# noamzilo/sed-crnn

Measured on AMD Instinct MI355X. Metric: mel-frames/sec training throughput (seq=256, mel=40), higher is better.
Workload: dtype f32; 1 GPU; BASELINE config 2: mono (B=128,256,40,1) per GPU, 3xConv3x3(128)+BN+ReLU+pool(1,2)+dropout0.5, BiGRU 2x128, Linear(256,1), BCEWithLogits, Adam lr 1e-3; full fit step (fwd+loss+bwd+allreduce+Adam); global_batch=128, seq_len=256, n_mels=40, parallelism=single

## Files before the change

### include/sedcrnn.h

```cpp
#ifndef SEDCRNN_H
#define SEDCRNN_H

#include <stddef.h>
#include <stdint.h>

#ifdef __cplusplus
extern "C" {
#endif

#define SED_MAX_CONV 4
#define SED_MAX_GRU 4
#define SED_MAX_DENSE 4

int sed_version(void);
const char* sed_last_error_string(void);

int sed_conv3x3_pack_weights(const float* w_oihw, float* wp_fwd, float* wp_dgrad,
                             int Cout, int Cin, void* stream);

int sed_conv3x3_stat_rows(int B, int Cin, int F, int T, int Cout, int x_is_nchw);

int sed_conv3x3_plan(int B, int Cin, int F, int T, int Cout, int x_is_nchw, int which, int* out);

int sed_conv3x3_fwd(const float* x, int x_is_nchw, const float* wp, const float* bias,
// ... 130 lines not shown
                        void* workspace, int B, int Cin, int F, int T, int C, float drop_p,
                        const float* gamma, const float* beta, float* dgamma, void* stream);
int sed_conv1_bwd_wgrad_assemble(const float* partials, int rows, const double* moments, const float* wp, const float* bias,
                                 const float* mean, const float* rstd, const float* scale, const float* sum_g,
                                 const float* sum_gx, float* dw_oihw, float* dbias, int B, int Cin, int F, int T, int C,
                                 const float* gamma, const float* beta, float* dgamma, void* stream);

int sed_gemm_f32(const float* A, long a_si, long a_sk, const float* B, long b_sk, long b_sj,
                 float* C, long ldc, const float* bias, float beta, int M, int N, int K, void* stream);
size_t sed_gemm_f32_workspace_bytes(int M, int N, int K);
int sed_gemm_f32_ws(const float* A, long a_si, long a_sk, const float* B, long b_sk, long b_sj,
                    float* C, long ldc, const float* bias, int M, int N, int K, void* workspace, void* stream);

int sed_gemm_bf16_nt(const void* A, const void* B, const float* bias, float* C, long ldc, int M, int N, int K, void* stream);

int sed_gemm_f32_wgrad(const float* A, long a_si, long a_sk, const float* B, long b_sk, long b_sj,
                       float* C, long ldc, int M, int N, int K, void* workspace, void* stream);
int sed_gemm_f32_plan(int M, int N, int K, int policy, int* bm, int* bn, int* splits, int* k_len);

int sed_linear_fwd(const float* x, const float* W, const float* b, float* y,
                   int M, int K, int N, int relu, void* stream);
size_t sed_linear_bwd_workspace_bytes(int M, int K, int N);
int sed_linear_bwd(const float* x, const float* W, const float* y, float* dy, float* dx,
                   float* dW, float* db, void* workspace, int M, int K, int N, int relu, void* stream);

size_t sed_gru_seq_workspace_bytes(int H);
int sed_gru_seq_fwd(const float* gi, const float* const* whh, const float* const* bhh,
                    float* out, float* saved, void* workspace, int B, int T, int H, void* stream);
size_t sed_gru_seq_bwd_workspace_bytes(int B, int H);
int sed_gru_seq_bwd(const float* dout, const float* saved, const float* const* whh,
                    float* dgi, float* dgh, float* const* dbih, float* const* dbhh, void* workspace,
                    int B, int T, int H, void* stream);
int sed_gru_seq_variant(int B, int H, int* bt, int* hreg, int* hlds);

int sed_loss_fwd_bwd(const float* logits, const float* targets, int n, int kind, float alpha,
                     float gamma, int reduction_mean, float* loss, float* dlogits, float* probs,
                     void* stream);
int sed_sigmoid(const float* x, float* y, int n, void* stream);
int sed_scale(float* x, long n, float alpha, void* stream);

size_t sed_sqnorm_workspace_bytes(long n);
int sed_grad_norm_clip_coef(const float* g, long n, float max_norm, float* norm_out,
                            void* workspace, void* stream);
int sed_adam_step(float* p, const float* g, float* m, float* v, long n, float lr, float beta1,
                  float beta2, float eps, float weight_decay, int step, const float* grad_scale,
                  const uint64_t* step_state, void* stream);
int sed_step_advance(uint64_t* step_state, void* stream);

size_t sed_logmel_tables_bytes(const float* melfb_host, int n_fft, int n_mels);
int sed_logmel_build_tables(const float* window_host, const float* melfb_host, int n_fft, int n_mels,
                            void* tables_host, size_t tables_bytes);
int sed_logmel(const float* pcm, long n_samples, const void* tables, size_t tables_bytes,
               const float* mu, const float* inv_sigma, float* out,
               int n_fft, int hop, int n_mels, int pad_mode, void* stream);
size_t sed_logmel_batch_workspace_bytes(int R);
int sed_logmel_batch(const float* pcm, long pcm_len, const long* clips_host, int R, const void* tables, size_t tables_bytes,
                     const float* mu, const float* inv_sigma, float* out, long out_rows, int n_fft, int hop, int n_mels,
                     int pad_mode, void* workspace, size_t workspace_bytes, void* stream);
size_t sed_logmel_multi_workspace_bytes(int R, int channels);
int sed_logmel_multi(const float* pcm, long pcm_len, const long* clips_host, int R, int channels, const void* tables,
                     size_t tables_bytes, const float* mu, const float* inv_sigma, float* out, long out_rows, int n_fft, int hop,
                     int n_mels, int pad_mode, void* workspace, size_t workspace_bytes, void* stream);
size_t sed_logmel_gcc_workspace_bytes(int R, int channels);
int sed_logmel_gcc(const float* pcm, long pcm_len, const long* clips_host, int R, int channels, const void* tables,
                   size_t tables_bytes, const float* mu, const float* inv_sigma, float* out, long out_rows, int n_fft, int hop,
                   int n_mels, int n_lags, int pad_mode, void* workspace, size_t workspace_bytes, void* stream);
// ... 327 lines not shown
```

### sed_crnn_amd/_lib.py

```python
import ctypes as C
import os

HERE = os.path.dirname(os.path.abspath(__file__))
LIB_PATH = os.environ.get("SED_CRNN_LIB") or os.path.join(HERE, "libsedcrnn.so")

SED_MAX_CONV = 4
SED_MAX_GRU = 4
SED_MAX_DENSE = 4

_fp = C.c_void_p
_stream = C.c_void_p


class NetCfg(C.Structure):
    _fields_ = [
        ("B", C.c_int), ("Cin", C.c_int), ("F", C.c_int), ("T", C.c_int),
        ("n_conv", C.c_int),
        ("C", C.c_int * SED_MAX_CONV),
        ("pool_f", C.c_int * SED_MAX_CONV), ("pool_t", C.c_int * SED_MAX_CONV),
        ("drop_p", C.c_float * SED_MAX_CONV),
        ("n_gru", C.c_int), ("H", C.c_int * SED_MAX_GRU),
        ("n_dense", C.c_int), ("D", C.c_int * SED_MAX_DENSE),
        ("bn_eps", C.c_float), ("bn_momentum", C.c_float),
        ("conv_mode", C.c_int),
# ... 64 lines not shown
    "sed_conv1_bwd_wgrad_assemble": (_i, [_fp, _i, _fp, _fp, _fp, _fp, _fp, _fp, _fp, _fp, _fp, _fp, _i, _i, _i, _i, _i, _fp, _fp, _fp, _stream]),
    "sed_conv1_route": (_i, [_fp, _fp, _fp, _fp, _fp, _fp, _i, _i, _i, _i, _i, _i, _i, _stream]),
    "sed_conv1_bwd_reduce": (_i, [_fp, _fp, _fp, _fp, _fp, _fp, _fp, _fp, _fp, _i, _i, _i, _i, _i, _i, _i, _f, _u64, _fp, _stream]),
    "sed_conv1_bwd_apply_workspace_bytes": (_sz, [_i, _i, _i, _i]),
    "sed_conv1_bwd_apply_wgrad": (_i, [_fp, _fp, _fp, _fp, _fp, _fp, _fp, _fp, _fp, _fp, _fp, _fp, _fp, _i, _i, _i, _i, _i, _i, _i, _f, _u64, _fp, _fp, _fp, _fp, _stream]),
    "sed_bn_finalize_train": (_i, [_fp, _i, _i, _d, _fp, _fp, _fp, _fp, _f, _f, _fp, _fp, _fp, _fp, _stream]),
    "sed_bn_stat_sums": (_i, [_fp, _i, _i, _fp, _stream]),
    "sed_bn_finalize_from_sums": (_i, [_fp, _i, _d, _fp, _fp, _fp, _fp, _f, _f, _fp, _fp, _fp, _fp, _stream]),
    "sed_bn_finalize_eval": (_i, [_fp, _fp, _fp, _fp, _f, _i, _fp, _fp, _stream]),
    "sed_bn_relu_pool_drop_fwd": (_i, [_fp, _fp, _fp, _fp, _i, _i, _i, _i, _i, _i, _i, _f, _u64, _fp, _stream]),
    "sed_bn_relu_pool_route": (_i, [_fp, _fp, _fp, _fp, _i, _i, _i, _i, _i, _i, _stream]),
    "sed_bn_bwd_rows": (_i, [_i, _i, _i]),
    "sed_bn_relu_pool_drop_bwd_reduce": (_i, [_fp, _fp, _fp, _fp, _fp, _fp, _fp, _i, _i, _i, _i, _i, _i, _i, _f, _u64, _fp, _stream]),
    "sed_bn_bwd_finalize": (_i, [_fp, _i, _i, _fp, _fp, _fp, _fp, _stream]),
    "sed_bn_bwd_finalize_small_gamma": (_i, [_fp, _i, _i, _fp, _fp, _fp, _fp, _fp, _fp, _fp, _fp, _fp, _fp, _fp, _fp, _fp, _i, _i, _i, _i, _i, _f, _stream]),
    "sed_bn_bwd_reduce_pooled_supported": (_i, [_i, _i, _i, _i, _i]),
    "sed_bn_bwd_reduce_pooled": (_i, [_fp, _fp, _fp, _fp, _fp, _fp, _fp, _fp, _fp, _fp, _i, _i, _i, _i, _i, _i, _i, _f, _stream]),
    "sed_bn_relu_pool_drop_bwd_apply": (_i, [_fp, _fp, _fp, _fp, _fp, _fp, _fp, _fp, _fp, _fp, _i, _i, _i, _i, _i, _i, _i, _f, _u64, _fp, _stream]),
    "sed_reduce_rows": (_i, [_fp, _i, _i, _i, _fp, _stream]),
    "sed_gemm_f32": (_i, [_fp, _l, _l, _fp, _l, _l, _fp, _l, _fp, _f, _i, _i, _i, _stream]),
    "sed_gemm_f32_workspace_bytes": (_sz, [_i, _i, _i]),
    "sed_gemm_f32_ws": (_i, [_fp, _l, _l, _fp, _l, _l, _fp, _l, _fp, _i, _i, _i, _fp, _stream]),
    "sed_gemm_bf16_nt": (_i, [_fp, _fp, _fp, _fp, _l, _i, _i, _i, _stream]),
    "sed_gemm_f32_wgrad": (_i, [_fp, _l, _l, _fp, _l, _l, _fp, _l, _i, _i, _i, _fp, _stream]),
    "sed_gemm_f32_plan": (_i, [_i, _i, _i, _i, C.POINTER(_i), C.POINTER(_i), C.POINTER(_i), C.POINTER(_i)]),
    "sed_linear_fwd": (_i, [_fp, _fp, _fp, _fp, _i, _i, _i, _i, _stream]),
    "sed_linear_bwd_workspace_bytes": (_sz, [_i, _i, _i]),
    "sed_linear_bwd": (_i, [_fp, _fp, _fp, _fp, _fp, _fp, _fp, _fp, _i, _i, _i, _i, _stream]),
    "sed_gru_seq_workspace_bytes": (_sz, [_i]),
    "sed_gru_seq_fwd": (_i, [_fp, _pp, _pp, _fp, _fp, _fp, _i, _i, _i, _stream]),
    "sed_gru_seq_bwd_workspace_bytes": (_sz, [_i, _i]),
    "sed_gru_seq_bwd": (_i, [_fp, _fp, _pp, _fp, _fp, _pp, _pp, _fp, _i, _i, _i, _stream]),
    "sed_gru_seq_variant": (_i, [_i, _i, C.POINTER(_i), C.POINTER(_i), C.POINTER(_i)]),
    "sed_loss_fwd_bwd": (_i, [_fp, _fp, _i, _i, _f, _f, _i, _fp, _fp, _fp, _stream]),
    "sed_sigmoid": (_i, [_fp, _fp, _i, _stream]),
    "sed_scale": (_i, [_fp, _l, _f, _stream]),
    "sed_sqnorm_workspace_bytes": (_sz, [_l]),
    "sed_grad_norm_clip_coef": (_i, [_fp, _l, _f, _fp, _fp, _stream]),
    "sed_adam_step": (_i, [_fp, _fp, _fp, _fp, _l, _f, _f, _f, _f, _f, _i, _fp, _fp, _stream]),
    "sed_step_advance": (_i, [_fp, _stream]),
    "sed_logmel_tables_bytes": (_sz, [_fp, _i, _i]),
    "sed_logmel_build_tables": (_i, [_fp, _fp, _i, _i, _fp, _sz]),
    "sed_logmel": (_i, [_fp, _l, _fp, _sz, _fp, _fp, _fp, _i, _i, _i, _i, _stream]),
    "sed_logmel_batch_workspace_bytes": (_sz, [_i]),
    "sed_logmel_batch": (_i, [_fp, _l, _fp, _i, _fp, _sz, _fp, _fp, _fp, _l, _i, _i, _i, _i, _fp, _sz, _stream]),
    "sed_logmel_multi_workspace_bytes": (_sz, [_i, _i]),
    "sed_logmel_multi": (_i, [_fp, _l, _fp, _i, _i, _fp, _sz, _fp, _fp, _fp, _l, _i, _i, _i, _i, _fp, _sz, _stream]),
    "sed_logmel_gcc_workspace_bytes": (_sz, [_i, _i]),
    "sed_logmel_gcc": (_i, [_fp, _l, _fp, _i, _i, _fp, _sz, _fp, _fp, _fp, _l, _i, _i, _i, _i, _i, _fp, _sz, _stream]),
    "sed_event_tdoa_workspace_bytes": (_sz, [_i, _i, _l, _l, _i, _i]),
    "sed_event_tdoa": (_i, [_fp, _l, _fp, _i, _i, _fp, _sz, _fp, _fp, _fp, _fp, _l, _i, _i, _i, _i, _i, _fp, _fp, _fp, _fp, _fp, _sz,
                            _stream]),
    "sed_stream_ring_write_workspace_bytes": (_sz, [_i]),
    "sed_stream_ring_write": (_i, [_fp, _l, _i, _l, _fp, _l, _fp, _fp, _sz, _stream]),
    "sed_event_tdoa_ring_workspace_bytes": (_sz, [_i, _i, _l, _l, _i, _i]),
    "sed_event_tdoa_ring": (_i, [_fp, _l, _l, _fp, _i, _i, _fp, _sz, _fp, _fp, _fp, _fp, _l, _i, _i, _i, _i, _i, _i, _fp, _fp, _fp, _fp,
                                 _fp, _sz, _stream]),
    "sed_event_doa_workspace_bytes": (_sz, [_i, _i, _l, _l, _i, _i]),
    "sed_event_doa": (_i, [_fp, _l, _fp, _i, _i, _fp, _sz, _fp, _fp, _fp, _fp, _l, _i, _i, _i, _i, _i, _fp, _fp, _fp, _fp, _fp, _i, _i,
                           _fp, _fp, _fp, _fp, _fp, _sz, _stream]),
    "sed_event_doa_ring_workspace_bytes": (_sz, [_i, _i, _l, _l, _i, _i]),
    "sed_event_doa_ring": (_i, [_fp, _l, _l, _fp, _i, _i, _fp, _sz, _fp, _fp, _fp, _fp, _l, _i, _i, _i, _i, _i, _i, _fp, _fp, _fp, _fp,
                                _fp, _i, _i, _fp, _fp, _fp, _fp, _fp, _sz, _stream]),
    "sed_event_doa_track_workspace_bytes": (_sz, [_i, _i, _l, _l, _i, _i, _i, _i, _i]),
    "sed_event_doa_track": (_i, [_fp, _l, _fp, _i, _i, _fp, _sz, _fp, _fp, _fp, _fp, _l, _i, _i, _i, _i, _i, _fp, _fp, _fp, _fp, _fp, _i,
                                 _i, _fp, _fp, _fp, _fp, _i, _fp, _fp, _fp, _fp, _fp, _fp, _fp, _fp, _sz, _stream]),
# ... 140 lines not shown
```

### sed_crnn_amd/csrc/gru.hip

```cpp
#include "common.h"

static inline int gru_bt(int H, int B) {
    int bt = B >= 512 ? 4 : (B >= 256 ? 2 : 1);
    if (H >= 128 && bt > 2) bt = 2;
    return bt;
}

__global__ void gru_pack_whh_t_k(const float* __restrict__ w0, const float* __restrict__ w1,
                                 float* __restrict__ wt, int H) {
    int i = blockIdx.x * blockDim.x + threadIdx.x;
    int n = 3 * H * H;
    if (i >= 2 * n) return;
    int dir = i / n, e = i - dir * n;
    int g = e / H, k = e - g * H;
    const float* w = dir ? w1 : w0;
    wt[(size_t)dir * n + (size_t)k * 3 * H + g] = w[e];
}

constexpr int gru_nt(int hreg) { return hreg > 0 ? ((3 * hreg + 63) / 64) * 64 : 1024; }

__device__ __forceinline__ float gru_dot4(float w0, float w1, float w2, float w3, const f32x4& h) {
    return fmaf(w3, h[3], fmaf(w2, h[2], fmaf(w0, h[0], w1 * h[1])));
}

template <int HREG, int GRU_BT, int HTOT = HREG, int HLDS = 0>
__global__ __launch_bounds__(gru_nt(HTOT)) void gru_seq_fwd_k(
    const float* __restrict__ gi, const float* __restrict__ wt, const float* __restrict__ bhh0,
    const float* __restrict__ bhh1, float* __restrict__ out, float* __restrict__ saved, int B, int T, int H) {
    extern __shared__ __attribute__((aligned(16))) float smem[];
    float* h_s = smem;
    float* gh_s = smem + GRU_BT * H;
    float* w_l = smem + GRU_BT * 4 * H;
    const int g = threadIdx.x;
    const int dir = blockIdx.y, b0 = blockIdx.x * GRU_BT;
    const int H3 = 3 * H;
    const float* wtd = wt + (size_t)dir * H3 * H;
    const float* bhh = dir ? bhh1 : bhh0;
    const bool row = g < H3;
    const bool gate = g < H;
    constexpr bool HYB = HTOT != HREG && HREG > 0;

    float wreg[HREG > 0 ? HREG : 1];
    if (HREG > 0 && row) {
#pragma unroll
        for (int k = 0; k < HREG; ++k) wreg[k] = wtd[(size_t)k * H3 + g];
    }
    if (HYB && row) {
        for (int j = 0; j < HLDS; ++j) w_l[j * H3 + g] = wtd[(size_t)(HREG + j) * H3 + g];
    }
    const float bias = row ? bhh[g] : 0.f;
    for (int i = g; i < GRU_BT * H; i += blockDim.x) h_s[i] = 0.f;
    __syncthreads();

    float gr[GRU_BT], gz[GRU_BT], gn[GRU_BT], nr[GRU_BT], nz[GRU_BT], nn[GRU_BT], mr[GRU_BT], mz[GRU_BT], mn[GRU_BT];
    auto fetch_gi = [&](int s, float* a, float* bq, float* c) {
        const int tt = dir ? (T - 1 - s) : s;
#pragma unroll
        for (int b = 0; b < GRU_BT; ++b) {
            int bg = b0 + b;
            if (gate && bg < B && s < T) {
                const float* p = gi + (((size_t)bg * T + tt) * 2 + dir) * H3;
                a[b] = p[g]; bq[b] = p[H + g]; c[b] = p[2 * H + g];
            } else { a[b] = bq[b] = c[b] = 0.f; }
        }
    };
    fetch_gi(0, gr, gz, gn);
    fetch_gi(1, nr, nz, nn);
    for (int s = 0; s < T; ++s) {
        const int tt = dir ? (T - 1 - s) : s;
        fetch_gi(s + 2, mr, mz, mn);
        if (row) {
            float acc[GRU_BT];
#pragma unroll
            for (int b = 0; b < GRU_BT; ++b) acc[b] = bias;
            if (HREG > 0) {
#pragma unroll
                for (int k = 0; k < HREG; k += 4) {
#pragma unroll
                    for (int b = 0; b < GRU_BT; ++b) {
                        f32x4 hv = *(const f32x4*)(h_s + b * H + k);
                        acc[b] += gru_dot4(wreg[k], wreg[k + 1], wreg[k + 2], wreg[k + 3], hv);
                    }
                }
            }
            if (HYB) {
#pragma unroll 4
                for (int j = 0; j < HLDS; j += 4) {
                    const float w0 = w_l[j * H3 + g], w1 = w_l[(j + 1) * H3 + g], w2 = w_l[(j + 2) * H3 + g], w3 = w_l[(j + 3) * H3 + g];
#pragma unroll
                    for (int b = 0; b < GRU_BT; ++b) {
                        f32x4 hv = *(const f32x4*)(h_s + b * H + HREG + j);
                        acc[b] += gru_dot4(w0, w1, w2, w3, hv);
                    }
                }
            }
            if (HREG == 0 || HYB) {
                for (int k = HYB ? HREG + HLDS : 0; k < H; k += 4) {
                    float w0 = wtd[(size_t)k * H3 + g], w1 = wtd[(size_t)(k + 1) * H3 + g];
                    float w2 = wtd[(size_t)(k + 2) * H3 + g], w3 = wtd[(size_t)(k + 3) * H3 + g];
#pragma unroll
                    for (int b = 0; b < GRU_BT; ++b) {
                        f32x4 hv = *(const f32x4*)(h_s + b * H + k);
                        acc[b] += gru_dot4(w0, w1, w2, w3, hv);
                    }
                }
            }
#pragma unroll
            for (int b = 0; b < GRU_BT; ++b) gh_s[b * H3 + g] = acc[b];
        }
        __syncthreads();
        if (gate) {
#pragma unroll
            for (int b = 0; b < GRU_BT; ++b) {
                int bg = b0 + b;
                float ghr = gh_s[b * H3 + g], ghz = gh_s[b * H3 + H + g], ghn = gh_s[b * H3 + 2 * H + g];
                float hp = h_s[b * H + g];
                float r = __fdividef(1.f, 1.f + __expf(-(gr[b] + ghr)));
                float z = __fdividef(1.f, 1.f + __expf(-(gz[b] + ghz)));
                float a = gn[b] + r * ghn;
                float e2 = __expf(-2.f * fabsf(a));
                float n = copysignf(__fdividef(1.f - e2, 1.f + e2), a);
                float hn = (1.f - z) * n + z * hp;
                h_s[b * H + g] = hn;
                if (bg < B) {
                    out[((size_t)bg * T + tt) * 2 * H + dir * H + g] = hn;
                    if (saved) {
                        float* sp = saved + ((((size_t)bg * T + tt) * 2 + dir) * 5) * H + g;
                        sp[0] = r; sp[H] = z; sp[2 * H] = n; sp[3 * H] = ghn; sp[4 * H] = hp;
                    }
                }
            }
        }
#pragma unroll
        for (int b = 0; b < GRU_BT; ++b) {
            gr[b] = nr[b]; gz[b] = nz[b]; gn[b] = nn[b];
            nr[b] = mr[b]; nz[b] = mz[b]; nn[b] = mn[b];
        }
        __syncthreads();
    }
}

template <int HREG, int GRU_BT, int HTOT = HREG, int HLDS = 0>
__global__ __launch_bounds__(gru_nt(HTOT)) void gru_seq_bwd_k(
    const float* __restrict__ dout, const float* __restrict__ saved, const float* __restrict__ whh0,
    const float* __restrict__ whh1, float* __restrict__ dgi, float* __restrict__ dgh, float* __restrict__ bpart,
    int B, int T, int H) {
    extern __shared__ __attribute__((aligned(16))) float smem[];
    const int H3 = 3 * H;
    float* dgh_s = smem;
    float* part_s = smem + GRU_BT * H3;
    float* w_l = smem + GRU_BT * 2 * H3;
    const int g = threadIdx.x;
    const int dir = blockIdx.y, b0 = blockIdx.x * GRU_BT;
    const float* whh = dir ? whh1 : whh0;
    const bool row = g < H3;
    const bool gate = g < H;
    const int p = g / H, k = g - p * H;
    constexpr bool HYB = HTOT != HREG && HREG > 0;

    float wreg[HREG > 0 ? HREG : 1];
    if (HREG > 0 && row) {
#pragma unroll
        for (int j = 0; j < HREG; ++j) wreg[j] = whh[((size_t)p * H + j) * H + k];
    }
    if (HYB && row) {
        for (int j = 0; j < HLDS; ++j) w_l[j * H3 + g] = whh[((size_t)p * H + HREG + j) * H + k];
    }
    for (int i = g; i < 3 * GRU_BT * H; i += blockDim.x) part_s[i] = 0.f;
    float dhc[GRU_BT];
#pragma unroll
    for (int b = 0; b < GRU_BT; ++b) dhc[b] = 0.f;
// ... 107 lines not shown
    float a = 0.f;
#pragma unroll 8
    for (int b = 0; b < nblk; ++b) a += bpart[((size_t)(b * 2 + dir) * 4 + c) * H + j];
    float* dbih = dir ? dbih1 : dbih0;
    float* dbhh = dir ? dbhh1 : dbhh0;
    if (c < 3) dbih[c * H + j] = a;
    if (c < 2) dbhh[c * H + j] = a;
    if (c == 3) dbhh[2 * H + j] = a;
}

static int gru_threads(int H) { return ((3 * H + 63) / 64) * 64; }
#define GRU_HR 96
#define GRU_HL 48
#define GRU_HR_FWD 116

extern "C" size_t sed_gru_seq_workspace_bytes(int H) { return (size_t)2 * 3 * H * H * sizeof(float); }

struct GruVariant { int bt, hreg, hlds; };
static inline GruVariant gru_variant(int H, int B, int hyb_hreg) {
    const int bt = gru_bt(H, B);
    if (H == 8 || H == 16 || H == 32 || H == 64 || H == 128) return {bt, H, 0};
    if (H == 256 && bt == 1) return {bt, hyb_hreg, GRU_HL};
    return {bt, 0, 0};
}

extern "C" int sed_gru_seq_variant(int B, int H, int* bt, int* hreg, int* hlds) {
    SED_REQUIRE(bt && hreg && hlds, "gru_seq_variant: null pointer");
    SED_REQUIRE(B > 0 && H > 0 && H % 4 == 0 && 3 * H <= 1024, "gru_seq_variant: H=%d must be a multiple of 4 and <= 341", H);
    const GruVariant v = gru_variant(H, B, GRU_HR_FWD);
    *bt = v.bt; *hreg = v.hreg; *hlds = v.hlds;
    return 0;
}

#define GRU_BT3(HR, KERNEL, ...)                                                              \
    if (v.bt == 1) KERNEL<HR, 1><<<grid, nt, lds, s>>>(__VA_ARGS__);                          \
    else if (v.bt == 2) KERNEL<HR, 2><<<grid, nt, lds, s>>>(__VA_ARGS__);                     \
    else KERNEL<HR, 4><<<grid, nt, lds, s>>>(__VA_ARGS__)
#define GRU_DISPATCH(KERNEL, ...)                                                             \
    if (v.hlds > 0) {                                                                         \
        KERNEL<GRU_HRX, 1, 256, GRU_HL><<<grid, nt, lds + (size_t)GRU_HL * 768 * sizeof(float), s>>>(__VA_ARGS__); \
    } else switch (v.hreg) {                                                                  \
        case 8: GRU_BT3(8, KERNEL, __VA_ARGS__); break;                                       \
        case 16: GRU_BT3(16, KERNEL, __VA_ARGS__); break;                                     \
        case 32: GRU_BT3(32, KERNEL, __VA_ARGS__); break;                                     \
        case 64: GRU_BT3(64, KERNEL, __VA_ARGS__); break;                                     \
        case 128:                                                                             \
            if (v.bt == 1) KERNEL<128, 1><<<grid, nt, lds, s>>>(__VA_ARGS__);                 \
            else KERNEL<128, 2><<<grid, nt, lds, s>>>(__VA_ARGS__);                           \
            break;                                                                            \
        default: GRU_BT3(0, KERNEL, __VA_ARGS__); break;                                      \
    }

static int gru_pack_whh(const float* const* whh, float* wt, int H, hipStream_t s) {
    int n = 2 * 3 * H * H;
    gru_pack_whh_t_k<<<cdiv(n, 256), 256, 0, s>>>(whh[0], whh[1], wt, H);
    SED_LAUNCH_CHECK("gru_pack_whh_t");
    return 0;
}

int sed_internal_gru_seq_fwd_packed(const float* gi, const float* wt, const float* const* bhh, float* out,
                                    float* saved, int B, int T, int H, void* stream) {
    SED_REQUIRE(gi && wt && bhh && out && bhh[0] && bhh[1], "gru_seq_fwd: null pointer");
    SED_REQUIRE(B > 0 && T > 0 && H > 0 && H % 4 == 0 && 3 * H <= 1024, "gru_seq_fwd: H=%d must be a multiple of 4 and <= 341", H);
    hipStream_t s = as_stream(stream);
    const GruVariant v = gru_variant(H, B, GRU_HR_FWD);
    dim3 grid(cdiv(B, v.bt), 2);
    int nt = gru_threads(H);
    size_t lds = (size_t)v.bt * 4 * H * sizeof(float);
    SedProfScope prof(SED_K_GRU_FWD, s, 2.0 * 2 * B * (double)T * 3 * H * H);
    if (v.hlds > 0)
        (void)hipFuncSetAttribute((const void*)gru_seq_fwd_k<GRU_HR_FWD, 1, 256, GRU_HL>, hipFuncAttributeMaxDynamicSharedMemorySize, 160 * 1024);
#define GRU_HRX GRU_HR_FWD
    GRU_DISPATCH(gru_seq_fwd_k, gi, wt, bhh[0], bhh[1], out, saved, B, T, H);
#undef GRU_HRX
    SED_LAUNCH_CHECK("gru_seq_fwd");
    return 0;
}

extern "C" int sed_gru_seq_fwd(const float* gi, const float* const* whh, const float* const* bhh, float* out,
                               float* saved, void* workspace, int B, int T, int H, void* stream) {
    SED_REQUIRE(gi && whh && bhh && out && workspace && whh[0] && whh[1] && bhh[0] && bhh[1], "gru_seq_fwd: null pointer");
    SED_REQUIRE(B > 0 && T > 0 && H > 0 && H % 4 == 0 && 3 * H <= 1024, "gru_seq_fwd: H=%d must be a multiple of 4 and <= 341", H);
    SED_TRY(gru_pack_whh(whh, (float*)workspace, H, as_stream(stream)));
    return sed_internal_gru_seq_fwd_packed(gi, (const float*)workspace, bhh, out, saved, B, T, H, stream);
}

extern "C" size_t sed_gru_seq_bwd_workspace_bytes(int B, int H) { return (size_t)cdiv(B, gru_bt(H, B)) * 2 * 4 * H * sizeof(float); }

int sed_internal_gru_seq_bwd_partials(const float* dout, const float* saved, const float* const* whh, float* dgi,
                                      float* dgh, float* bpart, int B, int T, int H, void* stream) {
    SED_REQUIRE(dout && saved && whh && whh[0] && whh[1] && dgi && dgh, "gru_seq_bwd: null pointer");
    SED_REQUIRE(B > 0 && T > 0 && H > 0 && H % 4 == 0 && 3 * H <= 1024, "gru_seq_bwd: H=%d must be a multiple of 4 and <= 341", H);
    hipStream_t s = as_stream(stream);
    const GruVariant v = gru_variant(H, B, GRU_HR);
    dim3 grid(cdiv(B, v.bt), 2);
    int nt = gru_threads(H);
    size_t lds = (size_t)v.bt * 6 * H * sizeof(float);
    SedProfScope prof(SED_K_GRU_BWD, s, 2.0 * 2 * B * (double)T * 3 * H * H);
    if (v.hlds > 0)
        (void)hipFuncSetAttribute((const void*)gru_seq_bwd_k<GRU_HR, 1, 256, GRU_HL>, hipFuncAttributeMaxDynamicSharedMemorySize, 160 * 1024);
#define GRU_HRX GRU_HR
    GRU_DISPATCH(gru_seq_bwd_k, dout, saved, whh[0], whh[1], dgi, dgh, bpart, B, T, H);
#undef GRU_HRX
    SED_LAUNCH_CHECK("gru_seq_bwd");
    return 0;
}
// ... 20 lines not shown
```

### sed_crnn_amd/ops.py

```python
import ctypes as C

import torch

from ._lib import check, lib, ptr, stream_ptr


def _f32c(t):
    assert t.is_cuda and t.dtype == torch.float32 and t.is_contiguous(), "expect contiguous fp32 CUDA tensor"
    return t


def conv3x3_pack(w, mode=0):
    Cout, Cin = w.shape[:2]
    wf = torch.empty(9, Cout, Cin, device=w.device)
    wd = torch.empty(9, Cin, Cout, device=w.device)
    check(lib().sed_conv3x3_pack_weights_ex(ptr(_f32c(w)), ptr(wf), ptr(wd), Cout, Cin, mode, stream_ptr()), "conv3x3_pack")
    return wf, wd


def conv3x3_fwd(x, wp, bias, x_is_nchw, want_stats=True, mode=0):
    if x_is_nchw:
        B, Cin, F, T = x.shape
    else:
        B, T, F, Cin = x.shape
# ... 260 lines not shown

def gru_seq_fwd(gi, whh, bhh, save=True):
    B, T, _, H3 = gi.shape
    H = H3 // 3
    out = torch.empty(B, T, 2 * H, device=gi.device)
    saved = torch.empty(B, T, 2, 5, H, device=gi.device) if save else None
    ws = torch.empty(lib().sed_gru_seq_workspace_bytes(H) // 4, device=gi.device)
    check(lib().sed_gru_seq_fwd(ptr(_f32c(gi)), _pp(whh), _pp(bhh), ptr(out), ptr(saved), ptr(ws), B, T, H,
                                stream_ptr()), "gru_seq_fwd")
    return out, saved


def gru_seq_bwd(dout, saved, whh, want_bias=False):
    B, T, H2 = dout.shape
    H = H2 // 2
    dgi = torch.empty(B, T, 2, 3 * H, device=dout.device)
    dgh = torch.empty(B, T, 2, 3 * H, device=dout.device)
    if not want_bias:
        check(lib().sed_gru_seq_bwd(ptr(_f32c(dout)), ptr(saved), _pp(whh), ptr(dgi), ptr(dgh), None, None, None,
                                    B, T, H, stream_ptr()), "gru_seq_bwd")
        return dgi, dgh
    dbih = [torch.empty(3 * H, device=dout.device) for _ in range(2)]
    dbhh = [torch.empty(3 * H, device=dout.device) for _ in range(2)]
    ws = torch.empty(lib().sed_gru_seq_bwd_workspace_bytes(B, H) // 4 + 1, device=dout.device)
    check(lib().sed_gru_seq_bwd(ptr(_f32c(dout)), ptr(saved), _pp(whh), ptr(dgi), ptr(dgh), _pp(dbih), _pp(dbhh),
                                ptr(ws), B, T, H, stream_ptr()), "gru_seq_bwd")
    return dgi, dgh, dbih, dbhh


def gru_seq_variant(B, H):
    bt, hreg, hlds = C.c_int(), C.c_int(), C.c_int()
    check(lib().sed_gru_seq_variant(B, H, C.byref(bt), C.byref(hreg), C.byref(hlds)), "gru_seq_variant")
    return bt.value, hreg.value, hlds.value


def loss_fwd_bwd(logits, targets, kind="bce", alpha=0.25, gamma=2.0, reduction="mean"):
    if kind not in ("bce", "focal"):
        raise ValueError(f"loss kind must be 'bce' or 'focal', got {kind!r}")
    if reduction not in ("mean", "sum"):
        raise ValueError(f"reduction must be 'mean' or 'sum' (the fused loss returns a scalar), got {reduction!r}")
    if logits.shape != targets.shape:
        raise ValueError(f"logits {tuple(logits.shape)} and targets {tuple(targets.shape)} differ in shape")
    n = logits.numel()
    loss = torch.empty(1, device=logits.device)
    d = torch.empty_like(logits)
    p = torch.empty_like(logits)
    check(lib().sed_loss_fwd_bwd(ptr(_f32c(logits)), ptr(_f32c(targets)), n, 0 if kind == "bce" else 1, alpha, gamma,
                                 int(reduction == "mean"), ptr(loss), ptr(d), ptr(p), stream_ptr()), "loss_fwd_bwd")
    return loss, d, p


def sigmoid(x):
    y = torch.empty_like(x)
    check(lib().sed_sigmoid(ptr(_f32c(x)), ptr(y), x.numel(), stream_ptr()), "sigmoid")
    return y


def grad_norm_clip_coef(g, max_norm):
    out = torch.empty(2, device=g.device)
    ws = torch.empty(lib().sed_sqnorm_workspace_bytes(g.numel()) // 4, device=g.device)
    check(lib().sed_grad_norm_clip_coef(ptr(g), g.numel(), float(max_norm), ptr(out), ptr(ws), stream_ptr()), "grad_norm")
    return out


def adam_step(p, g, m, v, lr, beta1, beta2, eps, weight_decay, step, grad_scale=None, step_state=None):
    check(lib().sed_adam_step(ptr(p), ptr(g), ptr(m), ptr(v), p.numel(), lr, beta1, beta2, eps, weight_decay, step,
# ... 46 lines not shown
```

Measured before the change: 6.012 million mel-frames/s.

## Stage GRU forward input gates through double-buffered LDS chunks

Adds a staged variant of the GRU sequence forward kernel for register-resident weights. It prefetches input-gate values for a chunk of timesteps into registers, commits them to a double-buffered LDS region, and reads them from LDS in the step loop. The aim is to take per-step global-memory latency for gi off the serial recurrence critical path. In exchange it uses more LDS, which may lower occupancy, and adds barriers at chunk boundaries. The staged path is on by default and can be toggled through a new API.

```diff
diff --git a/include/sedcrnn.h b/include/sedcrnn.h
--- a/include/sedcrnn.h
+++ b/include/sedcrnn.h
@@ -186,6 +186,8 @@
                     float* dgi, float* dgh, float* const* dbih, float* const* dbhh, void* workspace,
                     int B, int T, int H, void* stream);
 int sed_gru_seq_variant(int B, int H, int* bt, int* hreg, int* hlds);
+int sed_gru_seq_staging(int on);
+int sed_gru_seq_chunk(int B, int H, int* sc_fwd, int* sc_bwd);
 
 int sed_loss_fwd_bwd(const float* logits, const float* targets, int n, int kind, float alpha,
                      float gamma, int reduction_mean, float* loss, float* dlogits, float* probs,
diff --git a/sed_crnn_amd/_lib.py b/sed_crnn_amd/_lib.py
--- a/sed_crnn_amd/_lib.py
+++ b/sed_crnn_amd/_lib.py
@@ -120,6 +120,8 @@
     "sed_gru_seq_bwd_workspace_bytes": (_sz, [_i, _i]),
     "sed_gru_seq_bwd": (_i, [_fp, _fp, _pp, _fp, _fp, _pp, _pp, _fp, _i, _i, _i, _stream]),
     "sed_gru_seq_variant": (_i, [_i, _i, C.POINTER(_i), C.POINTER(_i), C.POINTER(_i)]),
+    "sed_gru_seq_staging": (_i, [_i]),
+    "sed_gru_seq_chunk": (_i, [_i, _i, C.POINTER(_i), C.POINTER(_i)]),
     "sed_loss_fwd_bwd": (_i, [_fp, _fp, _i, _i, _f, _f, _i, _fp, _fp, _fp, _stream]),
     "sed_sigmoid": (_i, [_fp, _fp, _i, _stream]),
     "sed_scale": (_i, [_fp, _l, _f, _stream]),
diff --git a/sed_crnn_amd/csrc/gru.hip b/sed_crnn_amd/csrc/gru.hip
--- a/sed_crnn_amd/csrc/gru.hip
+++ b/sed_crnn_amd/csrc/gru.hip
@@ -23,7 +23,16 @@
     return fmaf(w3, h[3], fmaf(w2, h[2], fmaf(w0, h[0], w1 * h[1])));
 }
 
-template <int HREG, int GRU_BT, int HTOT = HREG, int HLDS = 0>
+constexpr int gru_sc_fwd(int H, int bt) {
+    for (int sc = 8; sc >= 2; sc /= 2)
+        if ((size_t)(4 + 2 * sc * 3) * bt * H * sizeof(float) <= 64 * 1024) return sc;
+    return 0;
+}
+constexpr size_t gru_lds_fwd(int H, int bt, bool staged) {
+    return (size_t)(4 + (staged ? 2 * gru_sc_fwd(H, bt) * 3 : 0)) * bt * H * sizeof(float);
+}
+
+template <int HREG, int GRU_BT, int HTOT = HREG, int HLDS = 0, bool STAGED = false>
 __global__ __launch_bounds__(gru_nt(HTOT)) void gru_seq_fwd_k(
     const float* __restrict__ gi, const float* __restrict__ wt, const float* __restrict__ bhh0,
     const float* __restrict__ bhh1, float* __restrict__ out, float* __restrict__ saved, int B, int T, int H) {
@@ -31,6 +40,7 @@
     float* h_s = smem;
     float* gh_s = smem + GRU_BT * H;
     float* w_l = smem + GRU_BT * 4 * H;
+    static_assert(!STAGED || (HREG == HTOT && HREG > 0 && gru_sc_fwd(HTOT, GRU_BT) > 0), "staged: register-resident variants only");
     const int g = threadIdx.x;
     const int dir = blockIdx.y, b0 = blockIdx.x * GRU_BT;
     const int H3 = 3 * H;
@@ -52,91 +62,177 @@
     for (int i = g; i < GRU_BT * H; i += blockDim.x) h_s[i] = 0.f;
     __syncthreads();
 
-    float gr[GRU_BT], gz[GRU_BT], gn[GRU_BT], nr[GRU_BT], nz[GRU_BT], nn[GRU_BT], mr[GRU_BT], mz[GRU_BT], mn[GRU_BT];
-    auto fetch_gi = [&](int s, float* a, float* bq, float* c) {
-        const int tt = dir ? (T - 1 - s) : s;
-#pragma unroll
-        for (int b = 0; b < GRU_BT; ++b) {
-            int bg = b0 + b;
-            if (gate && bg < B && s < T) {
-                const float* p = gi + (((size_t)bg * T + tt) * 2 + dir) * H3;
-                a[b] = p[g]; bq[b] = p[H + g]; c[b] = p[2 * H + g];
-            } else { a[b] = bq[b] = c[b] = 0.f; }
+    if constexpr (STAGED) {
+        constexpr int SC = gru_sc_fwd(HTOT, GRU_BT);
+        float st[SC][GRU_BT];
+        auto fetch = [&](int c) {
+#pragma unroll
+            for (int i = 0; i < SC; ++i) {
+                const int s = c * SC + i, tt = dir ? (T - 1 - s) : s;
+#pragma unroll
+                for (int b = 0; b < GRU_BT; ++b) {
+                    const int bg = b0 + b;
+                    st[i][b] = (row && bg < B && s < T) ? gi[(((size_t)bg * T + tt) * 2 + dir) * H3 + g] : 0.f;
+                }
+            }
+        };
+        auto commit = [&](int c) {
+            float* d = w_l + (c & 1) * SC * GRU_BT * H3;
+            if (row) {
+#pragma unroll
+                for (int i = 0; i < SC; ++i)
+#pragma unroll
+                    for (int b = 0; b < GRU_BT; ++b) d[(i * GRU_BT + b) * H3 + g] = st[i][b];
+            }
+        };
+        fetch(0);
+        commit(0);
+        __syncthreads();
+        const int nch = (T + SC - 1) / SC;
+        for (int c = 0; c < nch; ++c) {
+            fetch(c + 1);
+            const float* gc = w_l + (c & 1) * SC * GRU_BT * H3;
+            const int send = (c * SC + SC < T) ? SC : T - c * SC;
+            for (int i = 0; i < send; ++i) {
+                const int s = c * SC + i, tt = dir ? (T - 1 - s) : s;
+                float gr[GRU_BT], gz[GRU_BT], gn[GRU_BT];
+                if (gate) {
+#pragma unroll
+                    for (int b = 0; b < GRU_BT; ++b) {
+                        const float* q = gc + (i * GRU_BT + b) * H3 + g;
+                        gr[b] = q[0]; gz[b] = q[H]; gn[b] = q[2 * H];
+                    }
+                }
+                if (row) {
+                    float acc[GRU_BT];
+#pragma unroll
+                    for (int b = 0; b < GRU_BT; ++b) acc[b] = bias;
+#pragma unroll
+                    for (int k = 0; k < HREG; k += 4) {
+#pragma unroll
+                        for (int b = 0; b < GRU_BT; ++b) {
+                            f32x4 hv = *(const f32x4*)(h_s + b * H + k);
+                            acc[b] += gru_dot4(wreg[k], wreg[k + 1], wreg[k + 2], wreg[k + 3], hv);
+                        }
+                    }
+#pragma unroll
+                    for (int b = 0; b < GRU_BT; ++b) gh_s[b * H3 + g] = acc[b];
+                }
+                __syncthreads();
+                if (gate) {
+#pragma unroll
+                    for (int b = 0; b < GRU_BT; ++b) {
+                        int bg = b0 + b;
+                        float ghr = gh_s[b * H3 + g], ghz = gh_s[b * H3 + H + g], ghn = gh_s[b * H3 + 2 * H + g];
+                        float hp = h_s[b * H + g];
+                        float r = __fdividef(1.f, 1.f + __expf(-(gr[b] + ghr)));
+                        float z = __fdividef(1.f, 1.f + __expf(-(gz[b] + ghz)));
+                        float a = gn[b] + r * ghn;
+                        float e2 = __expf(-2.f * fabsf(a));
+                        float n = copysignf(__fdividef(1.f - e2, 1.f + e2), a);
+                        float hn = (1.f - z) * n + z * hp;
+                        h_s[b * H + g] = hn;
+                        if (bg < B) {
+                            out[((size_t)bg * T + tt) * 2 * H + dir * H + g] = hn;
+                            if (saved) {
+                                float* sp = saved + ((((size_t)bg * T + tt) * 2 + dir) * 5) * H + g;
+                                sp[0] = r; sp[H] = z; sp[2 * H] = n; sp[3 * H] = ghn; sp[4 * H] = hp;
+                            }
+                        }
+                    }
+                }
+                __syncthreads();
+            }
+            commit(c + 1);
+            __syncthreads();
         }
-    };
-    fetch_gi(0, gr, gz, gn);
-    fetch_gi(1, nr, nz, nn);
-    for (int s = 0; s < T; ++s) {
-        const int tt = dir ? (T - 1 - s) : s;
-        fetch_gi(s + 2, mr, mz, mn);
-        if (row) {
-            float acc[GRU_BT];
-#pragma unroll
-            for (int b = 0; b < GRU_BT; ++b) acc[b] = bias;
-            if (HREG > 0) {
-#pragma unroll
-                for (int k = 0; k < HREG; k += 4) {
-#pragma unroll
-                    for (int b = 0; b < GRU_BT; ++b) {
-                        f32x4 hv = *(const f32x4*)(h_s + b * H + k);
-                        acc[b] += gru_dot4(wreg[k], wreg[k + 1], wreg[k + 2], wreg[k + 3], hv);
-                    }
-                }
-            }
-            if (HYB) {
-#pragma unroll 4
-                for (int j = 0; j < HLDS; j += 4) {
-                    const float w0 = w_l[j * H3 + g], w1 = w_l[(j + 1) * H3 + g], w2 = w_l[(j + 2) * H3 + g], w3 = w_l[(j + 3) * H3 + g];
-#pragma unroll
-                    for (int b = 0; b < GRU_BT; ++b) {
-                        f32x4 hv = *(const f32x4*)(h_s + b * H + HREG + j);
-                        acc[b] += gru_dot4(w0, w1, w2, w3, hv);
-                    }
-                }
-            }
-            if (HREG == 0 || HYB) {
-                for (int k = HYB ? HREG + HLDS : 0; k < H; k += 4) {
-                    float w0 = wtd[(size_t)k * H3 + g], w1 = wtd[(size_t)(k + 1) * H3 + g];
-                    float w2 = wtd[(size_t)(k + 2) * H3 + g], w3 = wtd[(size_t)(k + 3) * H3 + g];
-#pragma unroll
-                    for (int b = 0; b < GRU_BT; ++b) {
-                        f32x4 hv = *(const f32x4*)(h_s + b * H + k);
-                        acc[b] += gru_dot4(w0, w1, w2, w3, hv);
-                    }
-                }
-            }
-#pragma unroll
-            for (int b = 0; b < GRU_BT; ++b) gh_s[b * H3 + g] = acc[b];
-        }
-        __syncthreads();
-        if (gate) {
+    } else {
+        float gr[GRU_BT], gz[GRU_BT], gn[GRU_BT], nr[GRU_BT], nz[GRU_BT], nn[GRU_BT], mr[GRU_BT], mz[GRU_BT], mn[GRU_BT];
+        auto fetch_gi = [&](int s, float* a, float* bq, float* c) {
+            const int tt = dir ? (T - 1 - s) : s;
 #pragma unroll
             for (int b = 0; b < GRU_BT; ++b) {
                 int bg = b0 + b;
-                float ghr = gh_s[b * H3 + g], ghz = gh_s[b * H3 + H + g], ghn = gh_s[b * H3 + 2 * H + g];
-                float hp = h_s[b * H + g];
-                float r = __fdividef(1.f, 1.f + __expf(-(gr[b] + ghr)));
-                float z = __fdividef(1.f, 1.f + __expf(-(gz[b] + ghz)));
-                float a = gn[b] + r * ghn;
-                float e2 = __expf(-2.f * fabsf(a));
-                float n = copysignf(__fdividef(1.f - e2, 1.f + e2), a);
-                float hn = (1.f - z) * n + z * hp;
-                h_s[b * H + g] = hn;
-                if (bg < B) {
-                    out[((size_t)bg * T + tt) * 2 * H + dir * H + g] = hn;
-                    if (saved) {
-                        float* sp = saved + ((((size_t)bg * T + tt) * 2 + dir) * 5) * H + g;
-                        sp[0] = r; sp[H] = z; sp[2 * H] = n; sp[3 * H] = ghn; sp[4 * H] = hp;
-                    }
-                }
-            }
+                if (gate && bg < B && s < T) {
+                    const float* p = gi + (((size_t)bg * T + tt) * 2 + dir) * H3;
+                    a[b] = p[g]; bq[b] = p[H + g]; c[b] = p[2 * H + g];
+                } else { a[b] = bq[b] = c[b] = 0.f; }
+            }
+        };
+        fetch_gi(0, gr, gz, gn);
+        fetch_gi(1, nr, nz, nn);
+        for (int s = 0; s < T; ++s) {
+            const int tt = dir ? (T - 1 - s) : s;
+            fetch_gi(s + 2, mr, mz, mn);
+            if (row) {
+                float acc[GRU_BT];
+#pragma unroll
+                for (int b = 0; b < GRU_BT; ++b) acc[b] = bias;
+                if (HREG > 0) {
+#pragma unroll
+                    for (int k = 0; k < HREG; k += 4) {
+#pragma unroll
+                        for (int b = 0; b < GRU_BT; ++b) {
+                            f32x4 hv = *(const f32x4*)(h_s + b * H + k);
+                            acc[b] += gru_dot4(wreg[k], wreg[k + 1], wreg[k + 2], wreg[k + 3], hv);
+                        }
+                    }
+                }
+                if (HYB) {
+#pragma unroll 4
+                    for (int j = 0; j < HLDS; j += 4) {
+                        const float w0 = w_l[j * H3 + g], w1 = w_l[(j + 1) * H3 + g], w2 = w_l[(j + 2) * H3 + g], w3 = w_l[(j + 3) * H3 + g];
+#pragma unroll
+                        for (int b = 0; b < GRU_BT; ++b) {
+                            f32x4 hv = *(const f32x4*)(h_s + b * H + HREG + j);
+                            acc[b] += gru_dot4(w0, w1, w2, w3, hv);
+                        }
+                    }
+                }
+                if (HREG == 0 || HYB) {
+                    for (int k = HYB ? HREG + HLDS : 0; k < H; k += 4) {
+                        float w0 = wtd[(size_t)k * H3 + g], w1 = wtd[(size_t)(k + 1) * H3 + g];
+                        float w2 = wtd[(size_t)(k + 2) * H3 + g], w3 = wtd[(size_t)(k + 3) * H3 + g];
+#pragma unroll
+                        for (int b = 0; b < GRU_BT; ++b) {
+                            f32x4 hv = *(const f32x4*)(h_s + b * H + k);
+                            acc[b] += gru_dot4(w0, w1, w2, w3, hv);
+                        }
+                    }
+                }
+#pragma unroll
+                for (int b = 0; b < GRU_BT; ++b) gh_s[b * H3 + g] = acc[b];
+            }
+            __syncthreads();
+            if (gate) {
+#pragma unroll
+                for (int b = 0; b < GRU_BT; ++b) {
+                    int bg = b0 + b;
+                    float ghr = gh_s[b * H3 + g], ghz = gh_s[b * H3 + H + g], ghn = gh_s[b * H3 + 2 * H + g];
+                    float hp = h_s[b * H + g];
+                    float r = __fdividef(1.f, 1.f + __expf(-(gr[b] + ghr)));
+                    float z = __fdividef(1.f, 1.f + __expf(-(gz[b] + ghz)));
+                    float a = gn[b] + r * ghn;
+                    float e2 = __expf(-2.f * fabsf(a));
+                    float n = copysignf(__fdividef(1.f - e2, 1.f + e2), a);
+                    float hn = (1.f - z) * n + z * hp;
+                    h_s[b * H + g] = hn;
+                    if (bg < B) {
+                        out[((size_t)bg * T + tt) * 2 * H + dir * H + g] = hn;
+                        if (saved) {
+                            float* sp = saved + ((((size_t)bg * T + tt) * 2 + dir) * 5) * H + g;
+                            sp[0] = r; sp[H] = z; sp[2 * H] = n; sp[3 * H] = ghn; sp[4 * H] = hp;
+                        }
+                    }
+                }
+            }
+#pragma unroll
+            for (int b = 0; b < GRU_BT; ++b) {
+                gr[b] = nr[b]; gz[b] = nz[b]; gn[b] = nn[b];
+                nr[b] = mr[b]; nz[b] = mz[b]; nn[b] = mn[b];
+            }
+            __syncthreads();
         }
-#pragma unroll
-        for (int b = 0; b < GRU_BT; ++b) {
-            gr[b] = nr[b]; gz[b] = nz[b]; gn[b] = nn[b];
-            nr[b] = mr[b]; nz[b] = mz[b]; nn[b] = mn[b];
-        }
-        __syncthreads();
     }
 }
 
@@ -310,6 +406,22 @@
     return 0;
 }
 
+static int g_gru_staging = 1;
+extern "C" int sed_gru_seq_staging(int on) {
+    const int was = g_gru_staging;
+    g_gru_staging = on != 0;
+    return was;
+}
+
+extern "C" int sed_gru_seq_chunk(int B, int H, int* sc_fwd, int* sc_bwd) {
+    SED_REQUIRE(sc_fwd && sc_bwd, "gru_seq_chunk: null pointer");
+    SED_REQUIRE(B > 0 && H > 0 && H % 4 == 0 && 3 * H <= 1024, "gru_seq_chunk: H=%d must be a multiple of 4 and <= 341", H);
+    const GruVariant v = gru_variant(H, B, GRU_HR_FWD);
+    *sc_fwd = g_gru_staging && v.hreg == H ? gru_sc_fwd(H, v.bt) : 0;
+    *sc_bwd = 0;
+    return 0;
+}
+
 #define GRU_BT3(HR, KERNEL, ...)                                                              \
     if (v.bt == 1) KERNEL<HR, 1><<<grid, nt, lds, s>>>(__VA_ARGS__);                          \
     else if (v.bt == 2) KERNEL<HR, 2><<<grid, nt, lds, s>>>(__VA_ARGS__);                     \
@@ -344,12 +456,33 @@
     const GruVariant v = gru_variant(H, B, GRU_HR_FWD);
     dim3 grid(cdiv(B, v.bt), 2);
     int nt = gru_threads(H);
-    size_t lds = (size_t)v.bt * 4 * H * sizeof(float);
+    size_t lds = gru_lds_fwd(H, v.bt, false);
     SedProfScope prof(SED_K_GRU_FWD, s, 2.0 * 2 * B * (double)T * 3 * H * H);
     if (v.hlds > 0)
         (void)hipFuncSetAttribute((const void*)gru_seq_fwd_k<GRU_HR_FWD, 1, 256, GRU_HL>, hipFuncAttributeMaxDynamicSharedMemorySize, 160 * 1024);
 #define GRU_HRX GRU_HR_FWD
-    GRU_DISPATCH(gru_seq_fwd_k, gi, wt, bhh[0], bhh[1], out, saved, B, T, H);
+#define GRU_FWD_STAGED(HR, BT) \
+    gru_seq_fwd_k<HR, BT, HR, 0, true><<<grid, nt, gru_lds_fwd(HR, BT, true), s>>>(gi, wt, bhh[0], bhh[1], out, saved, B, T, H)
+#define GRU_FWD_STAGED_BT3(HR)                       \
+    if (v.bt == 1) GRU_FWD_STAGED(HR, 1);            \
+    else if (v.bt == 2) GRU_FWD_STAGED(HR, 2);       \
+    else GRU_FWD_STAGED(HR, 4)
+    if (g_gru_staging && v.hreg == H) {
+        switch (H) {
+            case 8: GRU_FWD_STAGED_BT3(8); break;
+            case 16: GRU_FWD_STAGED_BT3(16); break;
+            case 32: GRU_FWD_STAGED_BT3(32); break;
+            case 64: GRU_FWD_STAGED_BT3(64); break;
+            default:
+                if (v.bt == 1) GRU_FWD_STAGED(128, 1);
+                else GRU_FWD_STAGED(128, 2);
+                break;
+        }
+    } else {
+        GRU_DISPATCH(gru_seq_fwd_k, gi, wt, bhh[0], bhh[1], out, saved, B, T, H);
+    }
+#undef GRU_FWD_STAGED_BT3
+#undef GRU_FWD_STAGED
 #undef GRU_HRX
     SED_LAUNCH_CHECK("gru_seq_fwd");
     return 0;
diff --git a/sed_crnn_amd/ops.py b/sed_crnn_amd/ops.py
--- a/sed_crnn_amd/ops.py
+++ b/sed_crnn_amd/ops.py
@@ -316,6 +316,16 @@
     bt, hreg, hlds = C.c_int(), C.c_int(), C.c_int()
     check(lib().sed_gru_seq_variant(B, H, C.byref(bt), C.byref(hreg), C.byref(hlds)), "gru_seq_variant")
     return bt.value, hreg.value, hlds.value
+
+
+def gru_seq_staging(on):
+    return bool(lib().sed_gru_seq_staging(int(bool(on))))
+
+
+def gru_seq_chunk(B, H):
+    f, b = C.c_int(), C.c_int()
+    check(lib().sed_gru_seq_chunk(B, H, C.byref(f), C.byref(b)), "gru_seq_chunk")
+    return f.value, b.value
 
 
 def loss_fwd_bwd(logits, targets, kind="bce", alpha=0.25, gamma=2.0, reduction="mean"):
```

Result: no change. 6.017 million mel-frames/s, median of 5 (+0.1%).
